# mingfeisun/DeepMimic_mujoco

Measured on AMD Instinct MI355X. Metric: env-steps/sec, higher is better.
Workload: dtype f64

## Files before the change

### deepmimic_mujoco_amd/csrc/kernels_rollout.hip

```cpp
#define DM_NO_LAUNCH_KERNELS
#include "kernels.h"

using namespace dm;

__global__ __launch_bounds__(64) void k_rollout_packed(const DevModel<Real>* __restrict__ Mp, const Batch<Real>* __restrict__ Bp, const StepRow* __restrict__ rows,
                                                       int n_substeps, int first, int count, int T, dmp::PolicyArgs pa, long long* __restrict__ wave_clk) {
  __shared__ SlotOrOne<Real> u;
  __shared__ SlotTables tb;
  static_assert(sizeof(SlotOrOne<Real>) == sizeof(SlotShared<Real>) * SLOTS, "the one-env code's LDS fits into the four slots'");
  const bool policy_clobbers_kin = pa.P != nullptr && sizeof(((SlotShared<Real>*)0)->r1) < 464 * sizeof(float);
  const Batch<Real>& B = *Bp;
  const int lane = dmw::lane(), slot = lane >> 4;
  stage_slot_tables(tb, lane);
  const bool live = SLOTS * (int)blockIdx.x + slot < count;
  int envs4[SLOTS];
  dispatch_env<SLOTS>(B, first, count, SLOTS * (int)blockIdx.x, lane, blockIdx.x == 0, envs4);
  const int env = slot == 0 ? envs4[0] : slot == 1 ? envs4[1] : slot == 2 ? envs4[2] : envs4[3];
  const int envs[4] = {dmw::bcast_i(env, 0), dmw::bcast_i(env, 16), dmw::bcast_i(env, 32), dmw::bcast_i(env, 48)};
  const int lv = live ? 1 : 0;
  const bool wr[4] = {dmw::bcast_i(lv, 0) != 0, dmw::bcast_i(lv, 16) != 0, dmw::bcast_i(lv, 32) != 0, dmw::bcast_i(lv, 48) != 0};
  const size_t n = (size_t)B.n_envs;
  const long long t_enter = wave_clk ? dmw::clk() : 0;
#ifdef DM_ROLLOUT_PROF
  long long* prof_acc = wave_clk ? wave_clk + (size_t)blockIdx.x * 4 * dm::PROF_SLOTS : (long long*)nullptr;
  if (prof_acc && lane < 64) prof_acc[lane] = 0;
  dmw::sync_mem();
#else
  long long* prof_acc = nullptr;
#endif
  slot_rollout<Real, RESTEP_ROWS>(*Mp, B, u.sh, tb, u.one.s, u.one.x, env, lane, live, rows, n_substeps, T, [&](int t) {
    if (!pa.P) return;
    dmp::PolicyArgs p = pa;
    p.action = pa.action + (size_t)(t + 1) * n * NU; p.vpred = pa.vpred + (size_t)t * n; p.counter = pa.counter + (unsigned long long)t;
    dmw::sync();
    dmp::policy_wave4<Real>(p, envs, wr, lane, reinterpret_cast<char*>(&u.sh[0]), (unsigned)sizeof(SlotShared<Real>), (unsigned)(offsetof(SlotShared<Real>, qpos) + 7 * sizeof(Real)),
                            (unsigned)(offsetof(SlotShared<Real>, qvel) + 6 * sizeof(Real)), (unsigned)offsetof(SlotShared<Real>, r1));
  }, prof_acc, policy_clobbers_kin);
#ifdef DM_ROLLOUT_PROF
  if (prof_acc && lane == 0) prof_acc[31] = dmw::clk() - t_enter;
#else
  if (wave_clk && lane == 0) wave_clk[(size_t)blockIdx.x * dm::PROF_SLOTS + 5] = dmw::clk() - t_enter;
#endif
}
```

### deepmimic_mujoco_amd/csrc/slot_step.h

```cpp
#pragma once

#include "env_step.h"
#include "slot_kernel.h"

namespace dm {

template <class R> struct DofVec { R r[DOF_PASSES]; };

template <class R>
DM_DEV void slot_integrate_pos(SlotShared<R>& s, const DofVec<R>& x0q, int sl, R h) {
  const R q0 = dmw::row_bcast<3>(x0q.r[0]), q1 = dmw::row_bcast<4>(x0q.r[0]), q2 = dmw::row_bcast<5>(x0q.r[0]), q3 = dmw::row_bcast<6>(x0q.r[0]);
  if (sl < 3) s.qpos[sl] = x0q.r[0] + h * s.tau[sl];
  else if (sl == 3) {
    R ax[3] = {s.tau[3], s.tau[4], s.tau[5]}, q[4] = {q0, q1, q2, q3}, qr[4];
    const R angle = h * normalize3(ax);
    if (angle == R(0)) { qr[0] = 1; qr[1] = qr[2] = qr[3] = 0; } else axisangle2quat(qr, ax, angle);
    normalize4(q);
    quat_mul(q, q, qr);
    s.qpos[3] = q[0]; s.qpos[4] = q[1]; s.qpos[5] = q[2]; s.qpos[6] = q[3];
  } else if (sl >= 7) s.qpos[sl] = x0q.r[0] + h * s.tau[sl - 1];
#pragma unroll
  for (int c = 1; c < Q_PASSES; c++) { const int i = sl + SW * c; if (i < NQ) s.qpos[i] = x0q.r[c] + h * s.tau[i - 1]; }
}

template <class R, bool PROF = false, bool CARRY = false, int MAXR = 2 * SW>
DM_DEV void slot_rk4_step(const DevModel<R>& M, SlotShared<R>& s, const SlotTables& tb, int sl, int lane, const LaneTopo& lt, R* xip, int& ovf, long long* prof = 0) {
  const R h = M.timestep;
  const R A[3] = {R(0.5), R(0.5), R(1)};
  const R Bw[4] = {R(1) / 6, R(1) / 3, R(1) / 3, R(1) / 6};
  DofVec<R> x0q, x0v, vprev, aprev, sumv, suma;
#pragma unroll
  for (int c = 0; c < DOF_PASSES; c++) {
    const int i = sl + SW * c;
    x0q.r[c] = i < NQ ? s.qpos[i] : R(0);
    const R v0 = i < NV ? s.qvel[i] : R(0);
    x0v.r[c] = v0; vprev.r[c] = v0; aprev.r[c] = 0; sumv.r[c] = 0; suma.r[c] = 0;
  }
  dmw::sync();
  for (int i = 0; i < 4; i++) {
    if (i > 0) {
      const R cf = A[i - 1];
#pragma unroll
      for (int c = 0; c < DOF_PASSES; c++) { const int d = sl + SW * c; if (d < NV) s.tau[d] = cf * vprev.r[c]; }
      dmw::sync();
      slot_integrate_pos(s, x0q, sl, h);
#pragma unroll
      for (int c = 0; c < DOF_PASSES; c++) {
        const int d = sl + SW * c;
        if (d < NV) { const R vi = x0v.r[c] + h * (cf * aprev.r[c]); vprev.r[c] = vi; s.qvel[d] = vi; }
      }
      dmw::sync();
    }
    typedef decltype(dmw::park(R(0))) ParkedR;
    ParkedR pk[5][DOF_PASSES];
#pragma unroll
    for (int c = 0; c < DOF_PASSES; c++) { pk[0][c] = dmw::park(x0q.r[c]); pk[1][c] = dmw::park(x0v.r[c]); pk[2][c] = dmw::park(vprev.r[c]); pk[3][c] = dmw::park(sumv.r[c]); pk[4][c] = dmw::park(suma.r[c]); }
    slot_forward<R, PROF, CARRY, MAXR>(M, s, tb, sl, lane, lt, xip, ovf, (const DebugOut*)0, prof);
#pragma unroll
    for (int c = 0; c < DOF_PASSES; c++) { x0q.r[c] = dmw::unpark(pk[0][c]); x0v.r[c] = dmw::unpark(pk[1][c]); vprev.r[c] = dmw::unpark(pk[2][c]); sumv.r[c] = dmw::unpark(pk[3][c]); suma.r[c] = dmw::unpark(pk[4][c]); }
#pragma unroll
    for (int c = 0; c < DOF_PASSES; c++) {
      const int d = sl + SW * c;
      if (d < NV) { const R a = s.qd.o.qacc[d]; aprev.r[c] = a; sumv.r[c] += Bw[i] * vprev.r[c]; suma.r[c] += Bw[i] * a; }
    }
  }
#pragma unroll
  for (int c = 0; c < DOF_PASSES; c++) { const int d = sl + SW * c; if (d < NV) s.tau[d] = sumv.r[c]; }
  dmw::sync();
  slot_integrate_pos(s, x0q, sl, h);
#pragma unroll
  for (int c = 0; c < DOF_PASSES; c++) { const int d = sl + SW * c; if (d < NV) { s.qvel[d] = x0v.r[c] + h * suma.r[c]; s.qws[d] = aprev.r[c]; } }
  dmw::sync();
}

template <class R>
DM_DEV void slot_load_env(const DevModel<R>& M, const Batch<R>& B, SlotShared<R>& s, int env, int sl, bool live, const double* action) {
#pragma unroll
  for (int c = 0; c < Q_PASSES; c++) {
    const int i = sl + SW * c;
    if (i < NQ) s.qpos[i] = B.qpos[(size_t)env * NQ + i];
    if (i < NV) { s.qvel[i] = B.qvel[(size_t)env * NV + i]; s.qws[i] = B.qws[(size_t)env * NV + i]; s.act[i] = 0; }
  }
  if (sl == 0) { s.status = 0; s.nefc = 0; s.ncon = 0; s.solver_iter = 0; }
  dmw::sync();
  if (action) {
#pragma unroll
    for (int c = 0; c < HINGE_PASSES; c++) {
      const int u = sl + SW * c;
      if (u < NU) {
        R a = (R)action[(size_t)env * NU + u];
        if (B.action_mode == 1) {
          const int idx = B.frame_idx[env];
          a += R(0.8) * (B.mocap_cfg[(size_t)idx * NQ + 7 + u] - s.qpos[7 + u]);
        } else if (B.action_mode == 2) {
          const int idx = B.frame_idx[env];
          a += M.kp[u + 6] * (B.mocap_cfg[(size_t)idx * NQ + 7 + u] - s.qpos[7 + u]) + M.kd[u + 6] * (B.mocap_vel[(size_t)idx * NV + 6 + u] - s.qvel[6 + u]);
        }
        if (live) B.ctrl[(size_t)env * NU + u] = a;
        const int d = u + 6;
        s.act[d] = M.gear[d] * clampr(a, M.ctrl_lo[d], M.ctrl_hi[d]);
      }
    }
  }
  dmw::sync_mem();
}

template <class R>
DM_DEV void slot_spd_control(const DevModel<R>& M, const Batch<R>& B, SlotShared<R>& s, const SlotTables& tb, int env, int sl, const LaneTopo& lt, bool live,
                             const DofVec<R>& qbar, const DofVec<R>& vbar) {
  const R h = M.timestep;
#pragma unroll
  for (int c = 0; c < DOF_PASSES; c++) { const int d = sl + SW * c; if (d < NV) s.act[d] = 0; }
  dmw::sync();
  R xip[3];
  slot_kinematics(M, s, sl, lt, xip);
  slot_bias(M, s, tb, sl, lt);
  slot_mass_matrix<R, false, true>(M, s, tb, sl, lt, (const DebugOut*)0);
  R pd[DOF_PASSES], kd[DOF_PASSES];
#pragma unroll
  for (int c = 0; c < DOF_PASSES; c++) {
    const int d = sl + SW * c;
    pd[c] = 0; kd[c] = 0;
    if (d >= 6 && d < NV) {
      const R q = s.qpos[d + 1], v = s.qvel[d];
      kd[c] = M.kd[d];
      pd[c] = M.kp[d] * (qbar.r[c] - q - h * v) + kd[c] * (vbar.r[c] - v);
      s.tau[d] += pd[c];
    }
  }
  dmw::sync();
  {
    R x[1][NV];
#pragma unroll
    for (int d = 0; d < NV; d++) x[0][d] = s.tau[d];
    slot_solve_LT<1>(x, s.r2.qLD);
#pragma unroll
    for (int d = 0; d < NV; d++) { x[0][d] *= s.qd.o.dinv[d]; dmw::pin_value(x[0][d]); }
    solve_L(x[0], s.r2.qLD);
    if (sl == 0) {
#pragma unroll
      for (int d = 0; d < NV; d++) s.qd.o.qacc[d] = x[0][d];
    }
  }
  dmw::sync();
#pragma unroll
  for (int c = 0; c < DOF_PASSES; c++) {
    const int d = sl + SW * c;
    if (d >= 6 && d < NV) {
      const R g = M.gear[d];
      const R ct = (pd[c] - h * kd[c] * s.qd.o.qacc[d]) / g;
      if (live) B.ctrl[(size_t)env * NU + (d - 6)] = ct;
      s.act[d] = g * clampr(ct, M.ctrl_lo[d], M.ctrl_hi[d]);
    }
  }
  dmw::sync_mem();
}

template <class R>
DM_DEV void slot_store_state(const Batch<R>& B, SlotShared<R>& s, int env, int sl, bool live) {
  if (!live) return;
#pragma unroll
  for (int c = 0; c < Q_PASSES; c++) {
    const int i = sl + SW * c;
    if (i < NQ) B.qpos[(size_t)env * NQ + i] = s.qpos[i];
    if (i < NV) { B.qvel[(size_t)env * NV + i] = s.qvel[i]; B.qws[(size_t)env * NV + i] = s.qws[i]; }
  }
}

template <class R>
DM_DEV void slot_reset_env(const DevModel<R>& M, const Batch<R>& B, SlotShared<R>& s, int env, int sl, bool doit, int mode, int hard) {
  const int ep = B.episode[env];
  const int genv = B.env_offset + env;
  int idx = (int)(rng_uniform(B.seed, genv, ep, 0) * (double)B.n_frames);
  if (idx >= B.n_frames) idx = B.n_frames - 1;
  if (doit) {
#pragma unroll
    for (int c = 0; c < Q_PASSES; c++) {
      const int i = sl + SW * c;
      if (mode == 0) {
        if (i < NQ) s.qpos[i] = B.mocap_cfg[(size_t)idx * NQ + i];
        if (i < NV) s.qvel[i] = B.mocap_vel[(size_t)idx * NV + i];
      } else if (mode == 1) {
        if (i < NQ) s.qpos[i] = M.qpos0[i] + (R)((rng_uniform(B.seed, genv, ep, 1 + i) * 2.0 - 1.0) * 0.01);
        if (i < NV) s.qvel[i] = (R)((rng_uniform(B.seed, genv, ep, 64 + i) * 2.0 - 1.0) * 0.01);
      } else {
        if (i < NQ) s.qpos[i] = M.qpos0[i];
        if (i < NV) s.qvel[i] = 0;
      }
      if (hard && i < NV) s.qws[i] = 0;
    }
    if (hard && sl == 0) B.time[env] = 0;
  }
  dmw::sync_mem();
  if (doit && sl == 0) {
    B.episode[env] = ep + 1;
    if (mode == 0 || (mode == 1 && hard)) set_frame(B, env, idx); else B.cycle[env] = 0;
  }
}

template <class R>
DM_DEV R slot_imitation_reward(const DevModel<R>& M, const Batch<R>& B, SlotShared<R>& s, int sl, const LaneTopo& lt, const R* ref, R shx, R shy, const R* refv = nullptr) {
  R qloc[4], aloc[3][3], xip[3];
  slot_kinematics(M, s, sl, lt, xip, qloc, aloc);
  const bool v1 = refv != nullptr;
  const R* rv = v1 ? refv : ref;
  const R* P = B.imit_pdev;
  R rq[4] = {s.qpos[3], s.qpos[4], s.qpos[5], s.qpos[6]};
  normalize4(rq);
  R pose = 0, vel = 0, eff = 0, root = 0, mx = 0, my = 0, mz = 0;
  if (sl < 13) {
    const int g = sl - 1;
    const int da = dmw::launder(lt.dofadr), nd = dmw::launder(lt.dofnum);
    const bool isroot = sl == 0, ball = !isroot && nd == 3;
    const R* rquat = ref + (isroot ? 3 : 13 + 4 * g);
    const R ident[4] = {1, 0, 0, 0};
    R q0[4], q1[4];
    for (int k = 0; k < 4; k++) { q0[k] = isroot ? rq[k] : (ball ? qloc[k] : ident[k]); q1[k] = (isroot || ball) ? rquat[k] : ident[k]; }
    const R th = quat_diff_theta(q0, q1);
    R pe = v1 ? fabs(th) : th * th, ve = 0;
    if (isroot) {
      R wv[3];
      const R wloc[3] = {s.qvel[3], s.qvel[4], s.qvel[5]};
      quat_rot(wv, rq, wloc);
      R dv2 = 0, dp2 = 0;
      for (int k = 0; k < 3; k++) { const R a = rv[10 + k] - wv[k]; ve += v1 ? fabs(a) : a * a; const R c = ref[7 + k] - s.qvel[k]; dv2 += c * c; }
      const R p1[3] = {ref[0] + shx, ref[1] + shy, ref[2]};
      for (int k = 0; k < 3; k++) { const R a = s.qpos[k] - p1[k]; dp2 += v1 ? fabs(a) : a * a; }
      root = v1 ? dp2 : dp2 + R(0.1) * pe + R(0.01) * dv2 + R(0.001) * ve;
    } else if (ball) {
      R wl[3] = {0, 0, 0};
      for (int k = 0; k < 3; k++) { const R rate = s.qvel[da + k]; wl[0] += aloc[k][0] * rate; wl[1] += aloc[k][1] * rate; wl[2] += aloc[k][2] * rate; }
      for (int k = 0; k < 3; k++) { const R w = rv[61 + 3 * g + k] - wl[k]; ve += v1 ? fabs(w) : w * w; }
    } else {
      const R a = ref[13 + 4 * g] - s.qpos[da + 1], w = rv[61 + 3 * g] - s.qvel[da];
      pe = v1 ? fabs(a) : a * a; ve = v1 ? fabs(w) + fabs(rv[61 + 3 * g + 1]) + fabs(rv[61 + 3 * g + 2]) : w * w;
    }
    const R wj = v1 ? (isroot ? R(1) : P[g] / P[12]) : P[isroot ? 12 : g];
    pose = wj * pe; vel = v1 ? ve : wj * ve;
  }
  if (sl < 4) {
    const int e = sl, b = (int)P[16 + e];
    const R ex[3] = {1, 0, 0};
    R fwd[3], p[3], rel[3];
    quat_rot(fwd, rq, ex);
    const R hn = sqrt(fwd[0] * fwd[0] + fwd[1] * fwd[1]);
    const R c = hn > R(0) ? fwd[0] / hn : R(1), sn = hn > R(0) ? fwd[1] / hn : R(0);
    mat_vec(p, s.xmat[b], P + 20 + 3 * e);
    for (int k = 0; k < 3; k++) { p[k] += s.xpos[b][k]; rel[k] = p[k] - s.qpos[k]; }
    rel[2] = p[2];
    const R f0[3] = {c * rel[0] + sn * rel[1], -sn * rel[0] + c * rel[1], rel[2]};
    for (int k = 0; k < 3; k++) { const R a = ref[97 + 3 * e + k] - f0[k]; eff += a * a; }
  }
#pragma unroll
  for (int cpass = 0; cpass < DOF_PASSES; cpass++) {
    const int d = sl + SW * cpass;
    if (d < NV) {
      const int b = TOPO.dof_body[d];
      const R* cb = s.r2.i.crb[b];
      const R* cd = s.cdof[d];
      const R qd = s.qvel[d], ms = cb[9];
      R axs[3];
      cross3(axs, cd, cb + 6);
      mx += qd * (ms * cd[3] + axs[0]); my += qd * (ms * cd[4] + axs[1]); mz += qd * (ms * cd[5] + axs[2]);
    }
  }
  pose = dmw::sum16(pose); vel = dmw::sum16(vel); eff = dmw::sum16(eff) / 4; root = dmw::row_bcast<0>(root);
  mx = dmw::sum16(mx) / M.total_mass; my = dmw::sum16(my) / M.total_mass; mz = dmw::sum16(mz) / M.total_mass;
  const R dc[3] = {ref[109] - mx, ref[110] - my, ref[111] - mz};
  const R com = R(0.1) * dot3(dc, dc);
  const R arg = sl == 0 ? R(-2) * pose : sl == 1 ? R(-0.1) * vel : sl == 2 ? (v1 ? R(-5) * root : R(-40) * eff) : sl == 3 ? R(-5) * root : R(-10) * com;
  const R wgt = sl == 0 ? R(0.5) : sl == 1 ? R(0.05) : sl == 2 ? (v1 ? R(0.2) : R(0.15)) : sl == 3 ? R(0.2) : R(0.1);
  R term = 0;
  if (sl < (v1 ? 3 : 5)) term = wgt * exp_once(arg);
  return dmw::sum16(term);
}

template <class R, bool PROF, bool CARRY, int MAXR, bool SPD>
DM_DEV bool slot_env_step_impl(const DevModel<R>& M, const Batch<R>& B, SlotShared<R>& s, SlotTables& tb, int env, int sl, int lane, bool live,
                               const double* action, double* obs, double* reward, unsigned char* done, int n_substeps, int* redo_count, int* redo_list,
                               long long* prof_out = 0, bool kin_carry = false) {
  long long prof[32];
  for (int k = 0; k < 32; k++) prof[k] = 0;
  long long tstart = 0;
  if (PROF) tstart = dmw::clk();
  const LaneTopo lt = lane_topo(sl);
  if constexpr (CARRY) { if (!kin_carry && sl == 0) s.kin_ok() = R(0); }
  DofVec<R> qbar, vbar;
  if constexpr (SPD) {
    slot_load_env(M, B, s, env, sl, live, (const double*)0);
#pragma unroll
    for (int c = 0; c < DOF_PASSES; c++) {
      const int d = sl + SW * c;
      qbar.r[c] = 0; vbar.r[c] = 0;
      if (d >= 6 && d < NV) {
        const int u = d - 6;
        if (action) qbar.r[c] = (R)action[(size_t)env * NU + u];
        if (B.action_mode == 4) {
          const int idx = B.frame_idx[env];
          qbar.r[c] += B.mocap_cfg[(size_t)idx * NQ + 7 + u];
          vbar.r[c] = B.mocap_vel[(size_t)idx * NV + 6 + u];
        }
      }
    }
  } else
  slot_load_env(M, B, s, env, sl, live, action);
  R xip[3];
  int why = 0;
  for (int k = 0; k < n_substeps; k++) {
    if constexpr (SPD) slot_spd_control(M, B, s, tb, env, sl, lt, live, qbar, vbar);
    slot_rk4_step<R, PROF, CARRY, MAXR>(M, s, tb, sl, lane, lt, xip, why, prof);
  }
  const bool ovf = dmw::row_ballot(why != 0, lane) != 0u;
  if (dmw::ballot(ovf) != 0ull) {
    unsigned bits = 0;
    for (int r = 0; r < 5; r++) if (dmw::row_ballot(((why >> r) & 1) != 0, lane) != 0u) bits |= 1u << r;
    if (ovf && live && sl == 0) {
      if (redo_count) { const int k = dmw::global_counter_next(redo_count); redo_list[k] = env; }
      for (int r = 0; r < 5; r++) if ((bits >> r) & 1u) dmw::global_counter_next(B.redo_why + 1 + r);
    }
  }
  live = live && !ovf;
  const R mz = sl < NB - 1 ? M.body_mass[sl + 1] * xip[2] : R(0);
  const R z = dmw::sum16(mz) / M.total_mass;
  bool dn = (z < R(0.7)) || (z > R(2.0));
  if (live) {
    if (B.diag != 0) {
      if (sl < NB - 1) for (int k = 0; k < 3; k++) B.xipos[(size_t)env * NB * 3 + 3 * (sl + 1) + k] = xip[k];
      if (sl < 3) B.xipos[(size_t)env * NB * 3 + sl] = 0;
      const int nc = s.ncon;
      for (int k = sl; k < MAXEFC * 2; k += SW) {
        const int c = k >> 1;
        int gid = -1;
        if (c < nc && c < SLOT_MAXCON) { const auto& rec = M.pair_rec[s.r1.rw.coni[c] & 0xff]; gid = (k & 1) ? rec.g2 : rec.g1; }
        B.cong[(size_t)env * MAXEFC * 2 + k] = gid;
      }
    }
    if (sl == 0) { B.comz[env] = z; B.ncon[env] = s.ncon; B.nefc[env] = s.nefc; B.status[env] = s.status; B.solver_iter[env] = s.solver_iter; if constexpr (!CARRY) order_ticket(B, env, s.nefc, s.solver_iter); }
  }
  R rew = 1;
  if (B.reward_mode == REW_V3_CONFIG) {
    const int idx = B.frame_idx[env];
    R err = 0;
    for (int i = 7; i < NQ; i++) err += fabs(s.qpos[i] - B.mocap_cfg[(size_t)idx * NQ + i]);
    rew = exp_once(-err);
    dmw::sync_mem();
    if (live && sl == 0) B.frame_idx[env] = (idx + 1) % B.n_frames;
  } else if (B.reward_mode == REW_V2_POSE) {
    const int idx = B.frame_idx[env] + 1;
    const int im = (idx + B.frame_init[env]) % B.n_frames;
    R err = 0, acs = 0;
    for (int i = 3; i < NQ; i++) err += fabs(s.qpos[i] - B.mocap_cfg[(size_t)im * NQ + i]);
    for (int u = 0; u < NU; u++) { const R c = B.ctrl[(size_t)env * NU + u]; acs += c * c; }
    rew = exp_once(R(-2) * err) - R(0.1) * acs;
    dmw::sync_mem();
    if (live && sl == 0) B.frame_idx[env] = idx;
  } else if (B.reward_mode == REW_IMITATION) {
    int k = B.frame_idx[env] + 1, cyc = B.cycle[env];
    bool ended = false;
    if (k >= B.n_frames) { if (B.imit_params[15] != R(0)) { k = 0; cyc += 1; } else { k = B.n_frames - 1; ended = true; } }
    rew = slot_imitation_reward(M, B, s, sl, lt, B.imit_table + (size_t)k * IMIT_FEAT, cyc * B.imit_params[13], cyc * B.imit_params[14]);
    dn = dn || ended;
    dmw::sync_mem();
    if (live && sl == 0) { B.frame_idx[env] = k; B.cycle[env] = cyc; }
  } else if (B.reward_mode == REW_V1_QUAT) {
    const int idx = B.frame_idx[env] + 1;
    int upd = (int)floor(B.mocap_dt / (M.timestep * n_substeps));
    if (upd < 1) upd = 1;
    const int k = (idx / upd + B.frame_init[env]) % B.n_frames, kv = k + 1 < B.n_frames ? k + 1 : B.n_frames - 1;
    const R robs = slot_imitation_reward(M, B, s, sl, lt, B.imit_table + (size_t)k * IMIT_FEAT, R(0), R(0), B.imit_table + (size_t)kv * IMIT_FEAT);
    R acs = 0;
    for (int u = 0; u < NU; u++) { const R c = B.ctrl[(size_t)env * NU + u]; acs += c * c; }
    rew = (idx % upd == 0 ? robs : R(0)) - R(0.1) * acs;
    dmw::sync_mem();
    if (live && sl == 0) B.frame_idx[env] = idx;
  }
  if (live && sl == 0) { B.time[env] += M.timestep * n_substeps; reward[env] = rew; done[env] = dn ? 1 : 0; if (B.kin) B.kin_ok[env] = 0; }
  if (B.autoreset) {
    dmw::sync_mem();
    slot_reset_env(M, B, s, env, sl, dn && live, B.autoreset == 1 ? 0 : 1, 1);
  }
  if constexpr (CARRY) { if (sl == 0) s.kin_ok() = (B.reward_mode >= REW_IMITATION && !ovf && !(dn && B.autoreset != 0)) ? R(1) : R(0); }
  if (live) {
#pragma unroll
    for (int c = 0; c < (NOBS + SW - 1) / SW; c++) {
      const int o = sl + SW * c;
      if (o < 28) obs[(size_t)env * NOBS + o] = s.qpos[7 + o];
      else if (o < NOBS) obs[(size_t)env * NOBS + o] = s.qvel[6 + (o - 28)];
    }
  }
  slot_store_state(B, s, env, sl, live);
  if (PROF && lane == 0) {
    prof[5] = dmw::clk() - tstart;
    for (int k = 0; k < 32; k++) prof_out[k] = prof[k];
  }
  return live;
}
template <class R, bool PROF = false, bool CARRY = false, int MAXR = 2 * SW>
DM_DEV bool slot_env_step(const DevModel<R>& M, const Batch<R>& B, SlotShared<R>& s, SlotTables& tb, int env, int sl, int lane, bool live,
                          const double* action, double* obs, double* reward, unsigned char* done, int n_substeps, int* redo_count, int* redo_list,
                          long long* prof_out = 0, bool kin_carry = false) {
  if (B.action_mode >= 3) return slot_env_step_impl<R, PROF, CARRY, MAXR, true>(M, B, s, tb, env, sl, lane, live, action, obs, reward, done, n_substeps, redo_count, redo_list, prof_out, kin_carry);
  return slot_env_step_impl<R, PROF, CARRY, MAXR, false>(M, B, s, tb, env, sl, lane, live, action, obs, reward, done, n_substeps, redo_count, redo_list, prof_out, kin_carry);
}

#ifdef DM_STATIC_CALLS
#define DM_CALL_SLOT_PARAM , int* call_slot
#define DM_CALL_SLOT_TOUCH(v) (*call_slot = (v))
#define DM_CALL_SLOT_ARG , &call_slot_mem
#define DM_CALL_SLOT_DECL int call_slot_mem = 0; asm volatile("" :: "v"(&call_slot_mem) : "memory")
#define DM_CALL_SLOT_USE asm volatile("" :: "v"(call_slot_mem))
#else
#define DM_CALL_SLOT_PARAM
#define DM_CALL_SLOT_TOUCH(v) ((void)0)
#define DM_CALL_SLOT_ARG
#define DM_CALL_SLOT_DECL ((void)0)
#define DM_CALL_SLOT_USE ((void)0)
#endif
template <class R> union SlotOrOne {
  SlotShared<R> sh[SLOTS];
  struct { Shared<R> s; StepScratch<R> x; } one;
};
template <class R, int NR>
DM_DEV_CALL64 void restep_one_env(const DevModel<R>* M, const Batch<R>* B, Shared<R>* s, StepScratch<R>* x, int env, int lane, const double* action, double* obs,
                                    double* reward, unsigned char* done, int n_substeps DM_CALL_SLOT_PARAM) {
  DM_CALL_SLOT_TOUCH(0);
  using dmw::uniform_ptr; using dmw::in_lds; using dmw::in_global; using dmw::in_constant;
  const Batch<R> Bv = *in_constant(B);
  env_step_impl<R, NR, false, false>(*in_constant(M), global_members(Bv), *in_lds(uniform_ptr(s)), *in_lds(uniform_ptr(x)), dmw::uniform(env), lane, in_global(uniform_ptr(action)),
                  in_global(uniform_ptr(obs)), in_global(uniform_ptr(reward)), in_global(uniform_ptr(done)), dmw::uniform(n_substeps));
}
template <class R, int MAXR>
DM_DEV_CALL64 int slot_env_step_call(const DevModel<R>* M, const Batch<R>* B, SlotShared<R>* s, SlotTables* tb, int env, int sl, int lane, bool live,
                                     const double* action, double* obs, double* reward, unsigned char* done, int n_substeps, int kin_carry DM_CALL_SLOT_PARAM) {
  using dmw::uniform_ptr; using dmw::in_lds; using dmw::in_global; using dmw::in_constant;
  const Batch<R> Bv = *in_constant(B);
  SlotShared<R>& sr = *in_lds(s);
  DM_CALL_SLOT_TOUCH(env);
  const bool stored = slot_env_step_impl<R, false, true, MAXR, false>(*in_constant(M), global_members(Bv), sr, *in_lds(uniform_ptr(tb)), env, sl, lane, live, in_global(uniform_ptr(action)),
                                                          in_global(uniform_ptr(obs)), in_global(uniform_ptr(reward)), in_global(uniform_ptr(done)), dmw::uniform(n_substeps), (int*)0, (int*)0,
                                                          (long long*)0, dmw::uniform(kin_carry) != 0);
  return (stored ? 1 : 0) | (sr.nefc << 8);
}
#ifdef DM_ROLLOUT_PROF
template <class R, int MAXR>
DM_DEV_CALL64 int slot_env_step_call_prof(const DevModel<R>* M, const Batch<R>* B, SlotShared<R>* s, SlotTables* tb, int env, int sl, int lane, bool live,
                                          const double* action, double* obs, double* reward, unsigned char* done, int n_substeps, long long* prof_out, int kin_carry DM_CALL_SLOT_PARAM) {
  DM_CALL_SLOT_TOUCH(env);
  using dmw::uniform_ptr; using dmw::in_lds; using dmw::in_global; using dmw::in_constant;
  const Batch<R> Bv = *in_constant(B);
  SlotShared<R>& sr = *in_lds(s);
  const bool stored = slot_env_step_impl<R, true, true, MAXR, false>(*in_constant(M), global_members(Bv), sr, *in_lds(uniform_ptr(tb)), env, sl, lane, live, in_global(uniform_ptr(action)),
                                                         in_global(uniform_ptr(obs)), in_global(uniform_ptr(reward)), in_global(uniform_ptr(done)), dmw::uniform(n_substeps), (int*)0, (int*)0,
                                                         in_global(uniform_ptr(prof_out)), dmw::uniform(kin_carry) != 0);
  return (stored ? 1 : 0) | (sr.nefc << 8);
}
#endif
struct StepRow { const double* action; double* obs; double* reward; unsigned char* done; };
#ifndef DM_EXT_MARGIN
#define DM_EXT_MARGIN 9
#endif
constexpr int EXT_MARGIN = DM_EXT_MARGIN;
template <class R, int NR, class POLICY>
DM_DEV void slot_rollout(const DevModel<R>& M_in, const Batch<R>& B, SlotShared<R>* sh, SlotTables& tb, Shared<R>& one_s, StepScratch<R>& one_x,
                         int env, int lane, bool live, const StepRow* rows, int n_substeps, int T, POLICY&& policy, long long* prof_acc = 0, bool policy_clobbers_kin = false) {
  const int slot = lane >> 4, sl = lane & 15;
  int carry = 0;
  int last_rows = B.nefc[env];
  DM_CALL_SLOT_DECL;
  for (int t = 0; t < T; t++) {
    const DevModel<R>& M = *dmw::launder_uniform_ptr(&M_in);
    const StepRow row = rows[t];
    const double* a_t = row.action;
    double* o_t = row.obs;
    double* r_t = row.reward;
    unsigned char* d_t = row.done;
    const bool heavy = rows_max(last_rows) > 2 * SW - EXT_MARGIN;
    int ret;
#ifdef DM_ROLLOUT_PROF
    if (prof_acc) {
      ret = heavy ? slot_env_step_call_prof<R, SLOT_MAXROWS>(&M, &B, &sh[slot], &tb, env, sl, lane, live, a_t, o_t, r_t, d_t, n_substeps, prof_acc + 32, carry DM_CALL_SLOT_ARG)
                  : slot_env_step_call_prof<R, 2 * SW>(&M, &B, &sh[slot], &tb, env, sl, lane, live, a_t, o_t, r_t, d_t, n_substeps, prof_acc + 32, carry DM_CALL_SLOT_ARG);
      if (lane == 0) { for (int k = 0; k < 31; k++) prof_acc[k] += prof_acc[32 + k]; if (heavy) prof_acc[28] += 1; }
    } else
#endif
    ret = heavy ? slot_env_step_call<R, SLOT_MAXROWS>(&M, &B, &sh[slot], &tb, env, sl, lane, live, a_t, o_t, r_t, d_t, n_substeps, carry DM_CALL_SLOT_ARG)
                : slot_env_step_call<R, 2 * SW>(&M, &B, &sh[slot], &tb, env, sl, lane, live, a_t, o_t, r_t, d_t, n_substeps, carry DM_CALL_SLOT_ARG);
    const bool stored = (ret & 1) != 0;
    last_rows = (stored || !live) ? (ret >> 8) : SLOT_MAXROWS;
    const int need = (live && !stored) ? 1 : 0;
    bool any = false;
    for (int k = 0; k < SLOTS; k++) {
      if (dmw::bcast_i(need, SW * k) == 0) continue;
      any = true;
      const int e = dmw::bcast_i(env, SW * k);
      dmw::sync_mem();
      restep_one_env<R, NR>(&M, &B, &one_s, &one_x, e, lane, a_t, o_t, r_t, d_t, n_substeps DM_CALL_SLOT_ARG);
      if (lane == 0) dmw::global_counter_next(B.redo_why);
      dmw::sync_mem();
    }
    if (any) {
#pragma unroll
      for (int c = 0; c < (NOBS + SW - 1) / SW; c++) {
        const int o = sl + SW * c;
        if (o < 28) sh[slot].qpos[7 + o] = (R)o_t[(size_t)env * NOBS + o];
        else if (o < NOBS) sh[slot].qvel[6 + (o - 28)] = (R)o_t[(size_t)env * NOBS + o];
      }
      dmw::sync_mem();
    }
    DM_CALL_SLOT_USE;
    policy(t);
    carry = (any || policy_clobbers_kin) ? 0 : 1;
    dmw::sync_mem();
  }
}

}
```

Baseline: 20.62 million.

## Keep per-env episode state resident in LDS across rollout steps

Adds a per-slot LDS record (time, frame index, cycle, episode, frame_init) that persists across rollout steps. Env state stays in LDS instead of being reloaded from global each step, and global-memory fences are swapped for LDS-only barriers where no policy writes are pending. The change also preloads imitation reference rows into registers and skips the reset RNG when no lane resets. It adds feature flags and more LDS use, tight against the occupancy budget, and risks stale state if the global and LDS copies diverge.

New measurement: 20.75 million (median of 6 runs). Within noise of the previous version (+0.6%).

```diff
diff --git a/deepmimic_mujoco_amd/csrc/kernels_rollout.hip b/deepmimic_mujoco_amd/csrc/kernels_rollout.hip
--- a/deepmimic_mujoco_amd/csrc/kernels_rollout.hip
+++ b/deepmimic_mujoco_amd/csrc/kernels_rollout.hip
@@ -7,7 +7,9 @@
                                                        int n_substeps, int first, int count, int T, dmp::PolicyArgs pa, long long* __restrict__ wave_clk) {
   __shared__ SlotOrOne<Real> u;
   __shared__ SlotTables tb;
+  __shared__ SlotResident<Real> res[SLOTS];
   static_assert(sizeof(SlotOrOne<Real>) == sizeof(SlotShared<Real>) * SLOTS, "the one-env code's LDS fits into the four slots'");
+  static_assert(sizeof(SlotOrOne<Real>) + sizeof(SlotTables) + sizeof(res) <= 40 * 1024, "four workgroups per CU: the records come out of the 496 bytes to spare");
   const bool policy_clobbers_kin = pa.P != nullptr && sizeof(((SlotShared<Real>*)0)->r1) < 464 * sizeof(float);
   const Batch<Real>& B = *Bp;
   const int lane = dmw::lane(), slot = lane >> 4;
@@ -28,14 +30,14 @@
 #else
   long long* prof_acc = nullptr;
 #endif
-  slot_rollout<Real, RESTEP_ROWS>(*Mp, B, u.sh, tb, u.one.s, u.one.x, env, lane, live, rows, n_substeps, T, [&](int t) {
+  slot_rollout<Real, RESTEP_ROWS>(*Mp, B, u.sh, res, tb, u.one.s, u.one.x, env, lane, live, rows, n_substeps, T, [&](int t) {
     if (!pa.P) return;
     dmp::PolicyArgs p = pa;
     p.action = pa.action + (size_t)(t + 1) * n * NU; p.vpred = pa.vpred + (size_t)t * n; p.counter = pa.counter + (unsigned long long)t;
     dmw::sync();
     dmp::policy_wave4<Real>(p, envs, wr, lane, reinterpret_cast<char*>(&u.sh[0]), (unsigned)sizeof(SlotShared<Real>), (unsigned)(offsetof(SlotShared<Real>, qpos) + 7 * sizeof(Real)),
                             (unsigned)(offsetof(SlotShared<Real>, qvel) + 6 * sizeof(Real)), (unsigned)offsetof(SlotShared<Real>, r1));
-  }, prof_acc, policy_clobbers_kin);
+  }, prof_acc, policy_clobbers_kin, pa.P != nullptr);
 #ifdef DM_ROLLOUT_PROF
   if (prof_acc && lane == 0) prof_acc[31] = dmw::clk() - t_enter;
 #else
diff --git a/deepmimic_mujoco_amd/csrc/slot_step.h b/deepmimic_mujoco_amd/csrc/slot_step.h
--- a/deepmimic_mujoco_amd/csrc/slot_step.h
+++ b/deepmimic_mujoco_amd/csrc/slot_step.h
@@ -73,14 +73,29 @@
   dmw::sync();
 }
 
-template <class R>
-DM_DEV void slot_load_env(const DevModel<R>& M, const Batch<R>& B, SlotShared<R>& s, int env, int sl, bool live, const double* action) {
-#pragma unroll
-  for (int c = 0; c < Q_PASSES; c++) {
-    const int i = sl + SW * c;
-    if (i < NQ) s.qpos[i] = B.qpos[(size_t)env * NQ + i];
-    if (i < NV) { s.qvel[i] = B.qvel[(size_t)env * NV + i]; s.qws[i] = B.qws[(size_t)env * NV + i]; s.act[i] = 0; }
-  }
+template <class R> struct SlotResident { R time; int frame_idx, cycle, episode, frame_init; };
+#ifndef DM_RESIDENT
+#define DM_RESIDENT 7
+#endif
+static_assert(!((DM_RESIDENT) & 2) || ((DM_RESIDENT) & 1), "LDS-only hand-offs need resident state rows");
+constexpr bool RES_STATE = ((DM_RESIDENT) & 1) != 0, RES_FENCE = ((DM_RESIDENT) & 2) != 0, RES_RESET = ((DM_RESIDENT) & 4) != 0, RES_REFROW = ((DM_RESIDENT) & 8) != 0;
+template <bool RES> DM_DEV void slot_hand_off() { if (RES && RES_FENCE) dmw::sync(); else dmw::sync_mem(); }
+
+template <class R, bool RES = false>
+DM_DEV void slot_load_env(const DevModel<R>& M, const Batch<R>& B, SlotShared<R>& s, int env, int sl, bool live, const double* action, SlotResident<R>* rs = nullptr, bool resident = false) {
+  if (!(RES && RES_STATE) || !resident) {
+#pragma unroll
+    for (int c = 0; c < Q_PASSES; c++) {
+      const int i = sl + SW * c;
+      if (i < NQ) s.qpos[i] = B.qpos[(size_t)env * NQ + i];
+      if (i < NV) { s.qvel[i] = B.qvel[(size_t)env * NV + i]; s.qws[i] = B.qws[(size_t)env * NV + i]; }
+    }
+  }
+  if (!resident) {
+    if (RES && sl == 0) { rs->time = B.time[env]; rs->frame_idx = B.frame_idx[env]; rs->cycle = B.cycle[env]; rs->episode = B.episode[env]; rs->frame_init = B.frame_init[env]; }
+  }
+#pragma unroll
+  for (int c = 0; c < Q_PASSES; c++) { const int i = sl + SW * c; if (i < NV) s.act[i] = 0; }
   if (sl == 0) { s.status = 0; s.nefc = 0; s.ncon = 0; s.solver_iter = 0; }
   dmw::sync();
   if (action) {
@@ -90,10 +105,10 @@
       if (u < NU) {
         R a = (R)action[(size_t)env * NU + u];
         if (B.action_mode == 1) {
-          const int idx = B.frame_idx[env];
+          const int idx = RES ? rs->frame_idx : B.frame_idx[env];
           a += R(0.8) * (B.mocap_cfg[(size_t)idx * NQ + 7 + u] - s.qpos[7 + u]);
         } else if (B.action_mode == 2) {
-          const int idx = B.frame_idx[env];
+          const int idx = RES ? rs->frame_idx : B.frame_idx[env];
           a += M.kp[u + 6] * (B.mocap_cfg[(size_t)idx * NQ + 7 + u] - s.qpos[7 + u]) + M.kd[u + 6] * (B.mocap_vel[(size_t)idx * NV + 6 + u] - s.qvel[6 + u]);
         }
         if (live) B.ctrl[(size_t)env * NU + u] = a;
@@ -102,7 +117,7 @@
       }
     }
   }
-  dmw::sync_mem();
+  if (RES && RES_FENCE && B.reward_mode != REW_V2_POSE && B.reward_mode != REW_V1_QUAT) dmw::sync(); else dmw::sync_mem();
 }
 
 template <class R>
@@ -167,12 +182,15 @@
   }
 }
 
-template <class R>
-DM_DEV void slot_reset_env(const DevModel<R>& M, const Batch<R>& B, SlotShared<R>& s, int env, int sl, bool doit, int mode, int hard) {
-  const int ep = B.episode[env];
+template <class R, bool RES = false>
+DM_DEV void slot_reset_env(const DevModel<R>& M, const Batch<R>& B, SlotShared<R>& s, int env, int sl, bool doit, int mode, int hard, SlotResident<R>* rs = nullptr) {
+  int ep = 0, idx = 0;
   const int genv = B.env_offset + env;
-  int idx = (int)(rng_uniform(B.seed, genv, ep, 0) * (double)B.n_frames);
-  if (idx >= B.n_frames) idx = B.n_frames - 1;
+  if (!(RES && RES_RESET) || dmw::ballot(doit) != 0ull) {
+    ep = RES ? rs->episode : B.episode[env];
+    idx = (int)(rng_uniform(B.seed, genv, ep, 0) * (double)B.n_frames);
+    if (idx >= B.n_frames) idx = B.n_frames - 1;
+  }
   if (doit) {
 #pragma unroll
     for (int c = 0; c < Q_PASSES; c++) {
@@ -189,21 +207,38 @@
       }
       if (hard && i < NV) s.qws[i] = 0;
     }
-    if (hard && sl == 0) B.time[env] = 0;
-  }
-  dmw::sync_mem();
+    if (hard && sl == 0) { B.time[env] = 0; if (RES) rs->time = 0; }
+  }
+  slot_hand_off<RES>();
   if (doit && sl == 0) {
     B.episode[env] = ep + 1;
-    if (mode == 0 || (mode == 1 && hard)) set_frame(B, env, idx); else B.cycle[env] = 0;
-  }
-}
-
-template <class R>
+    if (RES) rs->episode = ep + 1;
+    if (mode == 0 || (mode == 1 && hard)) {
+      set_frame(B, env, idx);
+      if (RES) { rs->frame_init = idx; rs->frame_idx = (B.reward_mode == REW_V2_POSE || B.reward_mode == REW_V1_QUAT) ? 0 : idx; rs->cycle = 0; }
+    } else { B.cycle[env] = 0; if (RES) rs->cycle = 0; }
+  }
+}
+
+template <class R, bool PRE = false>
 DM_DEV R slot_imitation_reward(const DevModel<R>& M, const Batch<R>& B, SlotShared<R>& s, int sl, const LaneTopo& lt, const R* ref, R shx, R shy, const R* refv = nullptr) {
+  const bool v1 = refv != nullptr;
+  const R* rv = v1 ? refv : ref;
+  R f_q[4] = {0, 0, 0, 0}, f_w[3] = {0, 0, 0}, f_e[3] = {0, 0, 0}, f_c[3] = {0, 0, 0}, f_p[3] = {0, 0, 0}, f_v[3] = {0, 0, 0};
+  if constexpr (PRE) {
+    if (sl < 13) {
+      const R* a = ref + (sl == 0 ? 3 : 13 + 4 * (sl - 1));
+      const R* b = rv + (sl == 0 ? 10 : 61 + 3 * (sl - 1));
+      for (int k = 0; k < 4; k++) f_q[k] = a[k];
+      for (int k = 0; k < 3; k++) f_w[k] = b[k];
+    }
+    if (sl == 0) for (int k = 0; k < 3; k++) { f_p[k] = ref[k]; f_v[k] = ref[7 + k]; }
+    if (sl < 4) for (int k = 0; k < 3; k++) f_e[k] = ref[97 + 3 * sl + k];
+    for (int k = 0; k < 3; k++) f_c[k] = ref[109 + k];
+    dmw::sched_fence();
+  }
   R qloc[4], aloc[3][3], xip[3];
   slot_kinematics(M, s, sl, lt, xip, qloc, aloc);
-  const bool v1 = refv != nullptr;
-  const R* rv = v1 ? refv : ref;
   const R* P = B.imit_pdev;
   R rq[4] = {s.qpos[3], s.qpos[4], s.qpos[5], s.qpos[6]};
   normalize4(rq);
@@ -215,7 +250,7 @@
     const R* rquat = ref + (isroot ? 3 : 13 + 4 * g);
     const R ident[4] = {1, 0, 0, 0};
     R q0[4], q1[4];
-    for (int k = 0; k < 4; k++) { q0[k] = isroot ? rq[k] : (ball ? qloc[k] : ident[k]); q1[k] = (isroot || ball) ? rquat[k] : ident[k]; }
+    for (int k = 0; k < 4; k++) { q0[k] = isroot ? rq[k] : (ball ? qloc[k] : ident[k]); q1[k] = (isroot || ball) ? (PRE ? f_q[k] : rquat[k]) : ident[k]; }
     const R th = quat_diff_theta(q0, q1);
     R pe = v1 ? fabs(th) : th * th, ve = 0;
     if (isroot) {
@@ -223,17 +258,17 @@
       const R wloc[3] = {s.qvel[3], s.qvel[4], s.qvel[5]};
       quat_rot(wv, rq, wloc);
       R dv2 = 0, dp2 = 0;
-      for (int k = 0; k < 3; k++) { const R a = rv[10 + k] - wv[k]; ve += v1 ? fabs(a) : a * a; const R c = ref[7 + k] - s.qvel[k]; dv2 += c * c; }
-      const R p1[3] = {ref[0] + shx, ref[1] + shy, ref[2]};
+      for (int k = 0; k < 3; k++) { const R a = (PRE ? f_w[k] : rv[10 + k]) - wv[k]; ve += v1 ? fabs(a) : a * a; const R c = (PRE ? f_v[k] : ref[7 + k]) - s.qvel[k]; dv2 += c * c; }
+      const R p1[3] = {(PRE ? f_p[0] : ref[0]) + shx, (PRE ? f_p[1] : ref[1]) + shy, PRE ? f_p[2] : ref[2]};
       for (int k = 0; k < 3; k++) { const R a = s.qpos[k] - p1[k]; dp2 += v1 ? fabs(a) : a * a; }
       root = v1 ? dp2 : dp2 + R(0.1) * pe + R(0.01) * dv2 + R(0.001) * ve;
     } else if (ball) {
       R wl[3] = {0, 0, 0};
       for (int k = 0; k < 3; k++) { const R rate = s.qvel[da + k]; wl[0] += aloc[k][0] * rate; wl[1] += aloc[k][1] * rate; wl[2] += aloc[k][2] * rate; }
-      for (int k = 0; k < 3; k++) { const R w = rv[61 + 3 * g + k] - wl[k]; ve += v1 ? fabs(w) : w * w; }
+      for (int k = 0; k < 3; k++) { const R w = (PRE ? f_w[k] : rv[61 + 3 * g + k]) - wl[k]; ve += v1 ? fabs(w) : w * w; }
     } else {
-      const R a = ref[13 + 4 * g] - s.qpos[da + 1], w = rv[61 + 3 * g] - s.qvel[da];
-      pe = v1 ? fabs(a) : a * a; ve = v1 ? fabs(w) + fabs(rv[61 + 3 * g + 1]) + fabs(rv[61 + 3 * g + 2]) : w * w;
+      const R a = (PRE ? f_q[0] : ref[13 + 4 * g]) - s.qpos[da + 1], w = (PRE ? f_w[0] : rv[61 + 3 * g]) - s.qvel[da];
+      pe = v1 ? fabs(a) : a * a; ve = v1 ? fabs(w) + fabs(PRE ? f_w[1] : rv[61 + 3 * g + 1]) + fabs(PRE ? f_w[2] : rv[61 + 3 * g + 2]) : w * w;
     }
     const R wj = v1 ? (isroot ? R(1) : P[g] / P[12]) : P[isroot ? 12 : g];
     pose = wj * pe; vel = v1 ? ve : wj * ve;
@@ -249,7 +284,7 @@
     for (int k = 0; k < 3; k++) { p[k] += s.xpos[b][k]; rel[k] = p[k] - s.qpos[k]; }
     rel[2] = p[2];
     const R f0[3] = {c * rel[0] + sn * rel[1], -sn * rel[0] + c * rel[1], rel[2]};
-    for (int k = 0; k < 3; k++) { const R a = ref[97 + 3 * e + k] - f0[k]; eff += a * a; }
+    for (int k = 0; k < 3; k++) { const R a = (PRE ? f_e[k] : ref[97 + 3 * e + k]) - f0[k]; eff += a * a; }
   }
 #pragma unroll
   for (int cpass = 0; cpass < DOF_PASSES; cpass++) {
@@ -266,7 +301,7 @@
   }
   pose = dmw::sum16(pose); vel = dmw::sum16(vel); eff = dmw::sum16(eff) / 4; root = dmw::row_bcast<0>(root);
   mx = dmw::sum16(mx) / M.total_mass; my = dmw::sum16(my) / M.total_mass; mz = dmw::sum16(mz) / M.total_mass;
-  const R dc[3] = {ref[109] - mx, ref[110] - my, ref[111] - mz};
+  const R dc[3] = {(PRE ? f_c[0] : ref[109]) - mx, (PRE ? f_c[1] : ref[110]) - my, (PRE ? f_c[2] : ref[111]) - mz};
   const R com = R(0.1) * dot3(dc, dc);
   const R arg = sl == 0 ? R(-2) * pose : sl == 1 ? R(-0.1) * vel : sl == 2 ? (v1 ? R(-5) * root : R(-40) * eff) : sl == 3 ? R(-5) * root : R(-10) * com;
   const R wgt = sl == 0 ? R(0.5) : sl == 1 ? R(0.05) : sl == 2 ? (v1 ? R(0.2) : R(0.15)) : sl == 3 ? R(0.2) : R(0.1);
@@ -278,7 +313,8 @@
 template <class R, bool PROF, bool CARRY, int MAXR, bool SPD>
 DM_DEV bool slot_env_step_impl(const DevModel<R>& M, const Batch<R>& B, SlotShared<R>& s, SlotTables& tb, int env, int sl, int lane, bool live,
                                const double* action, double* obs, double* reward, unsigned char* done, int n_substeps, int* redo_count, int* redo_list,
-                               long long* prof_out = 0, bool kin_carry = false) {
+                               long long* prof_out = 0, bool kin_carry = false, SlotResident<R>* rs = nullptr, bool resident = false) {
+  constexpr bool RES = CARRY && !SPD;
   long long prof[32];
   for (int k = 0; k < 32; k++) prof[k] = 0;
   long long tstart = 0;
@@ -303,7 +339,7 @@
       }
     }
   } else
-  slot_load_env(M, B, s, env, sl, live, action);
+  slot_load_env<R, RES>(M, B, s, env, sl, live, action, rs, resident);
   R xip[3];
   int why = 0;
   for (int k = 0; k < n_substeps; k++) {
@@ -339,45 +375,52 @@
   }
   R rew = 1;
   if (B.reward_mode == REW_V3_CONFIG) {
-    const int idx = B.frame_idx[env];
+    const int idx = RES ? rs->frame_idx : B.frame_idx[env];
     R err = 0;
     for (int i = 7; i < NQ; i++) err += fabs(s.qpos[i] - B.mocap_cfg[(size_t)idx * NQ + i]);
     rew = exp_once(-err);
-    dmw::sync_mem();
+    slot_hand_off<RES>();
+    if (RES && sl == 0) rs->frame_idx = (idx + 1) % B.n_frames;
     if (live && sl == 0) B.frame_idx[env] = (idx + 1) % B.n_frames;
   } else if (B.reward_mode == REW_V2_POSE) {
-    const int idx = B.frame_idx[env] + 1;
-    const int im = (idx + B.frame_init[env]) % B.n_frames;
+    const int idx = (RES ? rs->frame_idx : B.frame_idx[env]) + 1;
+    const int im = (idx + (RES ? rs->frame_init : B.frame_init[env])) % B.n_frames;
     R err = 0, acs = 0;
     for (int i = 3; i < NQ; i++) err += fabs(s.qpos[i] - B.mocap_cfg[(size_t)im * NQ + i]);
     for (int u = 0; u < NU; u++) { const R c = B.ctrl[(size_t)env * NU + u]; acs += c * c; }
     rew = exp_once(R(-2) * err) - R(0.1) * acs;
-    dmw::sync_mem();
+    slot_hand_off<RES>();
+    if (RES && sl == 0) rs->frame_idx = idx;
     if (live && sl == 0) B.frame_idx[env] = idx;
   } else if (B.reward_mode == REW_IMITATION) {
-    int k = B.frame_idx[env] + 1, cyc = B.cycle[env];
+    int k = (RES ? rs->frame_idx : B.frame_idx[env]) + 1, cyc = RES ? rs->cycle : B.cycle[env];
     bool ended = false;
     if (k >= B.n_frames) { if (B.imit_params[15] != R(0)) { k = 0; cyc += 1; } else { k = B.n_frames - 1; ended = true; } }
-    rew = slot_imitation_reward(M, B, s, sl, lt, B.imit_table + (size_t)k * IMIT_FEAT, cyc * B.imit_params[13], cyc * B.imit_params[14]);
+    rew = slot_imitation_reward<R, RES && RES_REFROW>(M, B, s, sl, lt, B.imit_table + (size_t)k * IMIT_FEAT, cyc * B.imit_params[13], cyc * B.imit_params[14]);
     dn = dn || ended;
-    dmw::sync_mem();
+    slot_hand_off<RES>();
+    if (RES && sl == 0) { rs->frame_idx = k; rs->cycle = cyc; }
     if (live && sl == 0) { B.frame_idx[env] = k; B.cycle[env] = cyc; }
   } else if (B.reward_mode == REW_V1_QUAT) {
-    const int idx = B.frame_idx[env] + 1;
+    const int idx = (RES ? rs->frame_idx : B.frame_idx[env]) + 1;
     int upd = (int)floor(B.mocap_dt / (M.timestep * n_substeps));
     if (upd < 1) upd = 1;
-    const int k = (idx / upd + B.frame_init[env]) % B.n_frames, kv = k + 1 < B.n_frames ? k + 1 : B.n_frames - 1;
-    const R robs = slot_imitation_reward(M, B, s, sl, lt, B.imit_table + (size_t)k * IMIT_FEAT, R(0), R(0), B.imit_table + (size_t)kv * IMIT_FEAT);
+    const int k = (idx / upd + (RES ? rs->frame_init : B.frame_init[env])) % B.n_frames, kv = k + 1 < B.n_frames ? k + 1 : B.n_frames - 1;
+    const R robs = slot_imitation_reward<R, RES && RES_REFROW>(M, B, s, sl, lt, B.imit_table + (size_t)k * IMIT_FEAT, R(0), R(0), B.imit_table + (size_t)kv * IMIT_FEAT);
     R acs = 0;
     for (int u = 0; u < NU; u++) { const R c = B.ctrl[(size_t)env * NU + u]; acs += c * c; }
     rew = (idx % upd == 0 ? robs : R(0)) - R(0.1) * acs;
-    dmw::sync_mem();
+    slot_hand_off<RES>();
+    if (RES && sl == 0) rs->frame_idx = idx;
     if (live && sl == 0) B.frame_idx[env] = idx;
   }
+  if (RES) {
+    if (sl == 0) { const R tm = rs->time + M.timestep * n_substeps; rs->time = tm; if (live) { B.time[env] = tm; reward[env] = rew; done[env] = dn ? 1 : 0; if (B.kin) B.kin_ok[env] = 0; } }
+  } else
   if (live && sl == 0) { B.time[env] += M.timestep * n_substeps; reward[env] = rew; done[env] = dn ? 1 : 0; if (B.kin) B.kin_ok[env] = 0; }
   if (B.autoreset) {
-    dmw::sync_mem();
-    slot_reset_env(M, B, s, env, sl, dn && live, B.autoreset == 1 ? 0 : 1, 1);
+    slot_hand_off<RES>();
+    slot_reset_env<R, RES>(M, B, s, env, sl, dn && live, B.autoreset == 1 ? 0 : 1, 1, rs);
   }
   if constexpr (CARRY) { if (sl == 0) s.kin_ok() = (B.reward_mode >= REW_IMITATION && !ovf && !(dn && B.autoreset != 0)) ? R(1) : R(0); }
   if (live) {
@@ -431,27 +474,27 @@
 }
 template <class R, int MAXR>
 DM_DEV_CALL64 int slot_env_step_call(const DevModel<R>* M, const Batch<R>* B, SlotShared<R>* s, SlotTables* tb, int env, int sl, int lane, bool live,
-                                     const double* action, double* obs, double* reward, unsigned char* done, int n_substeps, int kin_carry DM_CALL_SLOT_PARAM) {
+                                     const double* action, double* obs, double* reward, unsigned char* done, int n_substeps, int kin_carry, SlotResident<R>* rs DM_CALL_SLOT_PARAM) {
   using dmw::uniform_ptr; using dmw::in_lds; using dmw::in_global; using dmw::in_constant;
   const Batch<R> Bv = *in_constant(B);
   SlotShared<R>& sr = *in_lds(s);
   DM_CALL_SLOT_TOUCH(env);
   const bool stored = slot_env_step_impl<R, false, true, MAXR, false>(*in_constant(M), global_members(Bv), sr, *in_lds(uniform_ptr(tb)), env, sl, lane, live, in_global(uniform_ptr(action)),
                                                           in_global(uniform_ptr(obs)), in_global(uniform_ptr(reward)), in_global(uniform_ptr(done)), dmw::uniform(n_substeps), (int*)0, (int*)0,
-                                                          (long long*)0, dmw::uniform(kin_carry) != 0);
+                                                          (long long*)0, (dmw::uniform(kin_carry) & 1) != 0, in_lds(rs), (dmw::uniform(kin_carry) & 2) != 0 && live);
   return (stored ? 1 : 0) | (sr.nefc << 8);
 }
 #ifdef DM_ROLLOUT_PROF
 template <class R, int MAXR>
 DM_DEV_CALL64 int slot_env_step_call_prof(const DevModel<R>* M, const Batch<R>* B, SlotShared<R>* s, SlotTables* tb, int env, int sl, int lane, bool live,
-                                          const double* action, double* obs, double* reward, unsigned char* done, int n_substeps, long long* prof_out, int kin_carry DM_CALL_SLOT_PARAM) {
+                                          const double* action, double* obs, double* reward, unsigned char* done, int n_substeps, long long* prof_out, int kin_carry, SlotResident<R>* rs DM_CALL_SLOT_PARAM) {
   DM_CALL_SLOT_TOUCH(env);
   using dmw::uniform_ptr; using dmw::in_lds; using dmw::in_global; using dmw::in_constant;
   const Batch<R> Bv = *in_constant(B);
   SlotShared<R>& sr = *in_lds(s);
   const bool stored = slot_env_step_impl<R, true, true, MAXR, false>(*in_constant(M), global_members(Bv), sr, *in_lds(uniform_ptr(tb)), env, sl, lane, live, in_global(uniform_ptr(action)),
                                                          in_global(uniform_ptr(obs)), in_global(uniform_ptr(reward)), in_global(uniform_ptr(done)), dmw::uniform(n_substeps), (int*)0, (int*)0,
-                                                         in_global(uniform_ptr(prof_out)), dmw::uniform(kin_carry) != 0);
+                                                         in_global(uniform_ptr(prof_out)), (dmw::uniform(kin_carry) & 1) != 0, in_lds(rs), (dmw::uniform(kin_carry) & 2) != 0 && live);
   return (stored ? 1 : 0) | (sr.nefc << 8);
 }
 #endif
@@ -460,11 +503,21 @@
 #define DM_EXT_MARGIN 9
 #endif
 constexpr int EXT_MARGIN = DM_EXT_MARGIN;
+static_assert(offsetof(SlotShared<double>, qws) + sizeof(((SlotShared<double>*)0)->qws) <= offsetof(SlotShared<double>, r1) &&
+              offsetof(SlotShared<double>, qvel) + sizeof(((SlotShared<double>*)0)->qvel) <= offsetof(SlotShared<double>, r1) &&
+              offsetof(SlotShared<double>, r1) + 464 * sizeof(float) <= offsetof(SlotShared<double>, nefc),
+              "float64 slots: the policy step's scratch (464 floats at r1) lies behind qpos / qvel / qws and inside the slot");
+static_assert(offsetof(SlotShared<float>, qws) + sizeof(((SlotShared<float>*)0)->qws) <= offsetof(SlotShared<float>, r1) &&
+              offsetof(SlotShared<float>, qvel) + sizeof(((SlotShared<float>*)0)->qvel) <= offsetof(SlotShared<float>, r1) &&
+              offsetof(SlotShared<float>, r1) + 464 * sizeof(float) <= offsetof(SlotShared<float>, nefc),
+              "float32 slots: the policy step's scratch (464 floats at r1) lies behind qpos / qvel / qws and inside the slot");
 template <class R, int NR, class POLICY>
-DM_DEV void slot_rollout(const DevModel<R>& M_in, const Batch<R>& B, SlotShared<R>* sh, SlotTables& tb, Shared<R>& one_s, StepScratch<R>& one_x,
-                         int env, int lane, bool live, const StepRow* rows, int n_substeps, int T, POLICY&& policy, long long* prof_acc = 0, bool policy_clobbers_kin = false) {
+DM_DEV void slot_rollout(const DevModel<R>& M_in, const Batch<R>& B, SlotShared<R>* sh, SlotResident<R>* res, SlotTables& tb, Shared<R>& one_s, StepScratch<R>& one_x,
+                         int env, int lane, bool live, const StepRow* rows, int n_substeps, int T, POLICY&& policy, long long* prof_acc = 0, bool policy_clobbers_kin = false,
+                         bool policy_writes = true) {
   const int slot = lane >> 4, sl = lane & 15;
   int carry = 0;
+  const bool fence_global = policy_writes || dmw::ballot(!live) != 0ull;
   int last_rows = B.nefc[env];
   DM_CALL_SLOT_DECL;
   for (int t = 0; t < T; t++) {
@@ -478,13 +531,13 @@
     int ret;
 #ifdef DM_ROLLOUT_PROF
     if (prof_acc) {
-      ret = heavy ? slot_env_step_call_prof<R, SLOT_MAXROWS>(&M, &B, &sh[slot], &tb, env, sl, lane, live, a_t, o_t, r_t, d_t, n_substeps, prof_acc + 32, carry DM_CALL_SLOT_ARG)
-                  : slot_env_step_call_prof<R, 2 * SW>(&M, &B, &sh[slot], &tb, env, sl, lane, live, a_t, o_t, r_t, d_t, n_substeps, prof_acc + 32, carry DM_CALL_SLOT_ARG);
+      ret = heavy ? slot_env_step_call_prof<R, SLOT_MAXROWS>(&M, &B, &sh[slot], &tb, env, sl, lane, live, a_t, o_t, r_t, d_t, n_substeps, prof_acc + 32, carry, &res[slot] DM_CALL_SLOT_ARG)
+                  : slot_env_step_call_prof<R, 2 * SW>(&M, &B, &sh[slot], &tb, env, sl, lane, live, a_t, o_t, r_t, d_t, n_substeps, prof_acc + 32, carry, &res[slot] DM_CALL_SLOT_ARG);
       if (lane == 0) { for (int k = 0; k < 31; k++) prof_acc[k] += prof_acc[32 + k]; if (heavy) prof_acc[28] += 1; }
     } else
 #endif
-    ret = heavy ? slot_env_step_call<R, SLOT_MAXROWS>(&M, &B, &sh[slot], &tb, env, sl, lane, live, a_t, o_t, r_t, d_t, n_substeps, carry DM_CALL_SLOT_ARG)
-                : slot_env_step_call<R, 2 * SW>(&M, &B, &sh[slot], &tb, env, sl, lane, live, a_t, o_t, r_t, d_t, n_substeps, carry DM_CALL_SLOT_ARG);
+    ret = heavy ? slot_env_step_call<R, SLOT_MAXROWS>(&M, &B, &sh[slot], &tb, env, sl, lane, live, a_t, o_t, r_t, d_t, n_substeps, carry, &res[slot] DM_CALL_SLOT_ARG)
+                : slot_env_step_call<R, 2 * SW>(&M, &B, &sh[slot], &tb, env, sl, lane, live, a_t, o_t, r_t, d_t, n_substeps, carry, &res[slot] DM_CALL_SLOT_ARG);
     const bool stored = (ret & 1) != 0;
     last_rows = (stored || !live) ? (ret >> 8) : SLOT_MAXROWS;
     const int need = (live && !stored) ? 1 : 0;
@@ -509,9 +562,18 @@
     }
     DM_CALL_SLOT_USE;
     policy(t);
-    carry = (any || policy_clobbers_kin) ? 0 : 1;
-    dmw::sync_mem();
-  }
-}
-
-}
+    carry = any ? 0 : (policy_clobbers_kin ? 2 : 3);
+    if (fence_global || !RES_FENCE) dmw::sync_mem();
+    else dmw::sync();
+  }
+}
+#if defined(DM_WAVE_TESTBENCH)
+template <class R, int NR, class POLICY>
+DM_DEV void slot_rollout(const DevModel<R>& M_in, const Batch<R>& B, SlotShared<R>* sh, SlotTables& tb, Shared<R>& one_s, StepScratch<R>& one_x,
+                         int env, int lane, bool live, const StepRow* rows, int n_substeps, int T, POLICY&& policy) {
+  static SlotResident<R> res[SLOTS];
+  slot_rollout<R, NR>(M_in, B, sh, res, tb, one_s, one_x, env, lane, live, rows, n_substeps, T, policy, (long long*)0, false, false);
+}
+#endif
+
+}
```
